# ethnhe/PVN3D

Measured on NVIDIA H100. Metric: frames/sec, higher is better.
Workload: dtype f32 (shared-MLP operands rounded to TF32, fp32 accumulate)

## Files before the change

pvn3d_b200/csrc/mlp_tc.cu:

```cuda
#include <cuda.h>

#include "common.cuh"

namespace pvn3d {
namespace {

constexpr int kMlpBM = 128;
constexpr int kMlpEpiWarps = 4;
constexpr int kMlpProWarps = 8;
constexpr int kMlpMmaWarps = 8;
constexpr int kMlpThreads = (kMlpEpiWarps + kMlpProWarps + kMlpMmaWarps) * 32;
constexpr int kMlpMaxStages = 6;
constexpr int kMlpSmemMax = 227 * 1024;

enum : int { PRO_DENSE = 0, PRO_FP_INTERP = 2, PRO_SA_FACT = 3, PRO_FP_FACT = 4 };
enum : int { EPI_STORE = 0, EPI_MAXPOOL = 1, EPI_SUMPOOL = 2, EPI_MAXPOOL_T = 3, EPI_STORE_T = 4 };

struct MlpArgs {
  alignas(64) CUtensorMap tmap;
  int use_tma;
  const float *w;
  const float *bias;
  long long rows;
  int k_pad;
// ... 816 lines not shown
  if (!enc || (reinterpret_cast<uintptr_t>(w) & 15u)) return false;
  const cuuint64_t dims[2] = {static_cast<cuuint64_t>(k_pad), static_cast<cuuint64_t>(n_pad)};
  const cuuint64_t strides[1] = {static_cast<cuuint64_t>(k_pad) * sizeof(float)};
  const cuuint32_t box[2] = {32u, static_cast<cuuint32_t>(bn)};
  const cuuint32_t estr[2] = {1u, 1u};
  return enc(map, CU_TENSOR_MAP_DATA_TYPE_FLOAT32, 2, const_cast<float *>(w), dims, strides, box, estr,
             CU_TENSOR_MAP_INTERLEAVE_NONE, CU_TENSOR_MAP_SWIZZLE_128B, CU_TENSOR_MAP_L2_PROMOTION_L2_256B,
             CU_TENSOR_MAP_FLOAT_OOB_FILL_NONE) == CUDA_SUCCESS;
}

template <int PRO, int EPI>
int launch_mlp(MlpArgs &a, cudaStream_t st) {
  if (a.rows <= 0) return PVN3D_OK;
  if (a.k_pad <= 0 || a.k_pad % 32 || a.n_pad <= 0 || a.n_pad % 16 || (reinterpret_cast<uintptr_t>(a.w) & 15u))
    return PVN3D_ERR_INVALID_ARG;
  a.bn = mma_n(a.n_pad);
  a.acc_ld = std::max(32, a.bn);
  const size_t stage_bytes = kMlpBM * 128 + align_up(static_cast<size_t>(a.bn) * 128, 1024);
  const size_t fixed = mlp_smem_front(0, a.bn, a.acc_ld) + kMlpEpiWarps * 4096 + sizeof(MlpSmemCtl);
  int stages = static_cast<int>((kMlpSmemMax - fixed) / stage_bytes);
  if (stages > kMlpMaxStages) stages = kMlpMaxStages;
  if (stages < 3) return PVN3D_ERR_UNSUPPORTED;
  a.stages = stages;
  const size_t smem = mlp_smem_front(stages, a.bn, a.acc_ld) + kMlpEpiWarps * 4096 + sizeof(MlpSmemCtl);
  a.use_tma = weight_tensor_map(&a.tmap, a.w, a.k_pad, a.n_pad, a.bn) ? 1 : 0;
  const int sms = std::max(1, sm_count() - a.reserve_sms);
  const long long tiles = ((a.rows + kMlpBM - 1) / kMlpBM) * ceil_div(a.n_pad, a.bn);
  auto kern = mlp_layer_kernel<PRO, EPI>;
  static PerDeviceOnce once;
  PVN3D_ONCE_PER_DEVICE(once, cudaFuncSetAttribute(kern, cudaFuncAttributeMaxDynamicSharedMemorySize, kMlpSmemMax),
                        "mlp smem attr");
  const unsigned grid = static_cast<unsigned>(std::min<long long>(tiles, sms));
  kern<<<grid, kMlpThreads, smem, st>>>(a);
  return check_launch("mlp_layer_kernel");
}

constexpr int kSa2Threads = (kMlpProWarps + kMlpMmaWarps) * 32;
constexpr int kSa2MaxStages = 8;
constexpr uint32_t kSa2StageBytes = kMlpBM * 128u;

struct Sa2Args {
  MlpArgs a;
  const float *w3, *bias3;
  int k3_pad, n3_pad;
};

struct Sa2SmemCtl {
  uint64_t full[kSa2MaxStages];
  uint64_t empty[kSa2MaxStages];
};

struct Sa2Smem {
  uint32_t w2, w3, h, ring, xchg, ctl, bytes;
};
static inline __host__ __device__ Sa2Smem sa2_smem(int k2_pad, int n2, int k3_pad, int n3, int stages) {
  Sa2Smem s;
  s.w2 = 0;
  s.w3 = s.w2 + static_cast<uint32_t>(k2_pad / 32) * static_cast<uint32_t>(n2) * 128u;
  s.h = s.w3 + static_cast<uint32_t>(k3_pad / 32) * static_cast<uint32_t>(n3) * 128u;
  s.ring = s.h + static_cast<uint32_t>(k3_pad / 32) * kMlpBM * 128u;
  s.xchg = s.ring + static_cast<uint32_t>(stages) * kSa2StageBytes;
  s.ctl = s.xchg + 4u * static_cast<uint32_t>(n3 > 32 ? n3 : 32) * 4u;
  s.bytes = 1024u + s.ctl + static_cast<uint32_t>(sizeof(Sa2SmemCtl));
  return s;
}

__device__ __forceinline__ void named_bar_sync(int id, int threads) {
  asm volatile("bar.sync %0, %1;" ::"r"(id), "r"(threads) : "memory");
}
__device__ __forceinline__ void named_bar_arrive(int id, int threads) {
  asm volatile("bar.arrive %0, %1;" ::"r"(id), "r"(threads) : "memory");
}

__device__ __forceinline__ void stage_weights(uint32_t dst, const float *w, int rows, int k_pad, int n) {
  const int per_chunk = n * 8;
  for (int i = threadIdx.x; i < (k_pad / 32) * per_chunk; i += blockDim.x) {
    const int kc = i / per_chunk, r = (i - kc * per_chunk) >> 3, c = i & 7;
    const float4 v = r < rows ? ldg128(w + static_cast<size_t>(r) * k_pad + kc * 32 + c * 4) : make_float4(0.f, 0.f, 0.f, 0.f);
    sts128(dst + static_cast<uint32_t>(kc * per_chunk) * 16u + sw128_off(r, c), v.x, v.y, v.z, v.w);
  }
}

template <int N2>
__device__ __forceinline__ void sa2_layer2(const Sa2Args &g, uint32_t ring, uint32_t w2_s, uint32_t h_s, int S,
                                           int it_base, int kc2, Sa2SmemCtl &ctl, unsigned wg, int frag_row,
                                           unsigned lane) {
  float d[N2 / 2];
#pragma unroll
  for (int i = 0; i < N2 / 2; ++i) d[i] = 0.f;
  int prev = -1;
  for (int kc = 0; kc < kc2; ++kc) {
    const int it = it_base + kc;
    const int s = it % S;
    mbar_wait(&ctl.full[s], static_cast<unsigned>((it / S) & 1));
    fence_proxy_async_smem();
    const uint64_t adesc = smem_desc_sw128(ring + static_cast<uint32_t>(s) * kSa2StageBytes + wg * 8192u);
    const uint64_t bdesc = smem_desc_sw128(w2_s + static_cast<uint32_t>(kc * N2) * 128u);
    wgmma_fence();
#pragma unroll
    for (int k4 = 0; k4 < 4; ++k4)
      wgmma_tf32<N2>(d, adesc + static_cast<uint64_t>(k4 * 2), bdesc + static_cast<uint64_t>(k4 * 2), (kc > 0 || k4 > 0) ? 1u : 0u);
    wgmma_commit();
    if (prev >= 0) {
      wgmma_wait<1>();
      if (lane == 0) mbar_arrive(&ctl.empty[prev]);
    }
    prev = s;
  }
  wgmma_wait<0>();
  acc_fence(d);
  if (lane == 0) mbar_arrive(&ctl.empty[prev]);
  named_bar_sync(1 + static_cast<int>(wg), 128);
  const int n2 = g.a.n_pad;
#pragma unroll
  for (int j = 0; j < N2 / 8; ++j) {
    if (8 * j >= g.k3_pad) break;
    const int c = 8 * j + 2 * static_cast<int>(lane & 3u);
    const float b0 = c < n2 ? __ldg(g.a.bias + c) : 0.f, b1 = c + 1 < n2 ? __ldg(g.a.bias + c + 1) : 0.f;
    const uint32_t off = static_cast<uint32_t>(c >> 5) * (kMlpBM * 128u) + static_cast<uint32_t>(frag_row) * 128u +
                         ((static_cast<uint32_t>(((c & 31) >> 2) ^ (frag_row & 7))) << 4) + (c & 3) * 4u;
    asm volatile("st.shared.v2.f32 [%0], {%1,%2};" ::"r"(h_s + off), "f"(to_tf32(fmaxf(d[4 * j] + b0, 0.f))),
                 "f"(to_tf32(fmaxf(d[4 * j + 1] + b1, 0.f)))
                 : "memory");
    asm volatile("st.shared.v2.f32 [%0], {%1,%2};" ::"r"(h_s + off + 8u * 128u), "f"(to_tf32(fmaxf(d[4 * j + 2] + b0, 0.f))),
                 "f"(to_tf32(fmaxf(d[4 * j + 3] + b1, 0.f)))
                 : "memory");
  }
  fence_proxy_async_smem();
  named_bar_sync(1 + static_cast<int>(wg), 128);
}

template <int HALF, int O, int NV>
__device__ __forceinline__ void rowmax_level(float (&p)[NV], unsigned lane) {
  if constexpr (HALF >= 1) {
    const bool hi = (lane & static_cast<unsigned>(O)) != 0;
#pragma unroll
    for (int i = 0; i < HALF; ++i) {
      const float keep = hi ? p[i + HALF] : p[i];
      const float send = hi ? p[i] : p[i + HALF];
      p[i] = fmaxf(keep, __shfl_xor_sync(0xffffffffu, send, O));
    }
  } else {
    p[0] = fmaxf(p[0], __shfl_xor_sync(0xffffffffu, p[0], O));
  }
}

template <int N3>
__global__ void __launch_bounds__(kSa2Threads, 1) mlp_sa_fact2_kernel(const __grid_constant__ Sa2Args g) {
  const MlpArgs &a = g.a;
  extern __shared__ unsigned char mlp_smem_raw[];
  const uint32_t raw = smem_u32(mlp_smem_raw);
  const uint32_t base = (raw + 1023u) & ~1023u;
  const int n2_mma = mma_n(a.n_pad);
  const int kc2 = a.k_pad / 32, kc3 = g.k3_pad / 32;
  const int S = a.stages;
  const Sa2Smem L = sa2_smem(a.k_pad, n2_mma, g.k3_pad, N3, S);
  Sa2SmemCtl &ctl = *reinterpret_cast<Sa2SmemCtl *>(mlp_smem_raw + (base - raw) + L.ctl);
  const int t = threadIdx.x;
  const unsigned warp = t >> 5, lane = t & 31u;
  const int tiles = static_cast<int>((a.rows + kMlpBM - 1) / kMlpBM);

  stage_weights(base + L.w2, a.w, a.n_pad, a.k_pad, n2_mma);
  stage_weights(base + L.w3, g.w3, g.n3_pad, g.k3_pad, N3);
  for (uint32_t i = t; i < static_cast<uint32_t>(kc3) * kMlpBM * 8u; i += kSa2Threads) sts128(base + L.h + i * 16u, 0.f, 0.f, 0.f, 0.f);
  if (t == 0) {
    for (int s = 0; s < S; ++s) {
      mbar_init(&ctl.full[s], 128);
      mbar_init(&ctl.empty[s], kMlpMmaWarps);
    }
    mbar_fence_init();
  }
  fence_proxy_async_smem();
  __syncthreads();

  if (warp < kMlpProWarps) {
    const int pt = t & 127;
    const unsigned grp = warp >> 2;
    const int pw = pt >> 5, sub = static_cast<int>(lane & 7u), rg = static_cast<int>(lane >> 3);
    const int r_first = 32 * pw + rg;
    int it_base = 0;
    for (int tile = blockIdx.x; tile < tiles; tile += gridDim.x, it_base += kc2) {
      if (kc2 == 1 && static_cast<unsigned>(it_base & 1) != grp) continue;
      const long long p_first = static_cast<long long>(tile) * kMlpBM + r_first;
      RowState rs;
      rows_setup<PRO_SA_FACT>(a, p_first, rs);
      for (int kc = 0; kc < kc2; ++kc) {
        const int it = it_base + kc;
        if (static_cast<unsigned>(it & 1) != grp) continue;
        const int s = static_cast<int>(it % S);
        mbar_wait(&ctl.empty[s], static_cast<unsigned>(((it / S) & 1) ^ 1));
        stage_a_chunk<PRO_SA_FACT>(a, rs, p_first, r_first, sub, kc * 32, base + L.ring + static_cast<uint32_t>(s) * kSa2StageBytes,
                                   true);
        fence_proxy_async_smem();
        mbar_arrive(&ctl.full[s]);
      }
    }
  } else {
    const unsigned mw = warp - kMlpProWarps, wg = mw >> 2, w4 = mw & 3u;
    const int frag_row = static_cast<int>(64 * wg + 16 * w4 + (lane >> 2));
    const uint32_t h_wg = base + L.h + wg * 8192u;
    const uint32_t xchg = base + L.xchg + (wg * 2u + (w4 >> 1)) * ((N3 > 32 ? N3 : 32) * 4u);
    constexpr int NV = N3 / 4;
    constexpr int NF = NV >= 8 ? NV / 8 : 1;
    int it_base = 0;
    for (int tile = blockIdx.x; tile < tiles; tile += gridDim.x, it_base += kc2) {
      const long long p0 = static_cast<long long>(tile) * kMlpBM;
      if (n2_mma == 16) sa2_layer2<16>(g, base + L.ring, base + L.w2, base + L.h, S, it_base, kc2, ctl, wg, frag_row, lane);
      else if (n2_mma == 32) sa2_layer2<32>(g, base + L.ring, base + L.w2, base + L.h, S, it_base, kc2, ctl, wg, frag_row, lane);
      else if (n2_mma == 64) sa2_layer2<64>(g, base + L.ring, base + L.w2, base + L.h, S, it_base, kc2, ctl, wg, frag_row, lane);
      else sa2_layer2<128>(g, base + L.ring, base + L.w2, base + L.h, S, it_base, kc2, ctl, wg, frag_row, lane);
      float d[N3 / 2];
#pragma unroll
      for (int i = 0; i < N3 / 2; ++i) d[i] = 0.f;
      wgmma_fence();
      for (int kc = 0; kc < kc3; ++kc) {
        const uint64_t adesc = smem_desc_sw128(h_wg + static_cast<uint32_t>(kc) * (kMlpBM * 128u));
        const uint64_t bdesc = smem_desc_sw128(base + L.w3 + static_cast<uint32_t>(kc * N3) * 128u);
#pragma unroll
        for (int k4 = 0; k4 < 4; ++k4)
          wgmma_tf32<N3>(d, adesc + static_cast<uint64_t>(k4 * 2), bdesc + static_cast<uint64_t>(k4 * 2), (kc > 0 || k4 > 0) ? 1u : 0u);
      }
      wgmma_commit();
      wgmma_wait<0>();
      acc_fence(d);
      float p[NV];
#pragma unroll
      for (int j = 0; j < N3 / 8; ++j) {
        p[2 * j] = fmaxf(d[4 * j], d[4 * j + 2]);
        p[2 * j + 1] = fmaxf(d[4 * j + 1], d[4 * j + 3]);
      }
      rowmax_level<NV / 2, 16>(p, lane);
      rowmax_level<NV / 4, 8>(p, lane);
      rowmax_level<NV / 8, 4>(p, lane);
      bool owner = true;
      long long grow = (p0 + 64 * wg + 16 * w4) / 16;
      if (a.pool == 32) {
        if (w4 & 1u) {
#pragma unroll
          for (int i = 0; i < NF; ++i)
            asm volatile("st.shared.f32 [%0], %1;" ::"r"(xchg + (lane * NF + i) * 4u), "f"(p[i]) : "memory");
          named_bar_arrive(3 + static_cast<int>(wg * 2 + (w4 >> 1)), 64);
          owner = false;
        } else {
          named_bar_sync(3 + static_cast<int>(wg * 2 + (w4 >> 1)), 64);
#pragma unroll
          for (int i = 0; i < NF; ++i) {
            float q;
            asm volatile("ld.shared.f32 %0, [%1];" : "=f"(q) : "r"(xchg + (lane * NF + i) * 4u) : "memory");
            p[i] = fmaxf(p[i], q);
          }
        }
        grow = (p0 + 64 * wg + 32 * (w4 >> 1)) / 32;
      }
      if (owner && grow * a.pool < a.rows && (NV >= 8 || !(lane & 4u))) {
        const unsigned b4 = (lane >> 4) & 1u, b3 = (lane >> 3) & 1u, b2 = (lane >> 2) & 1u;
        float *o = a.out + grow * a.ldo + a.col0;
#pragma unroll
        for (int i = 0; i < NF; ++i) {
          const int io = i + (b4 ? NV / 2 : 0) + (b3 && NV >= 4 ? NV / 4 : 0) + (b2 && NV >= 8 ? NV / 8 : 0);
          const int col = 8 * (io >> 1) + 2 * static_cast<int>(lane & 3u) + (io & 1);
          if (col < g.n3_pad) {
            float r = fmaxf(p[i] + __ldg(g.bias3 + col), 0.f);
            if (a.round_out) r = to_tf32(r);
            o[col] = r;
          }
        }
      }
    }
  }
}

int sa2_stages(int k2_pad, int n2_pad, int k3_pad, int n3_pad, int ns) {
  if ((ns != 16 && ns != 32) || n2_pad > 128 || n3_pad > 128) return 0;
  const uint32_t fixed = sa2_smem(k2_pad, mma_n(n2_pad), k3_pad, mma_n(n3_pad), 0).bytes;
  if (fixed >= static_cast<uint32_t>(kMlpSmemMax)) return 0;
  const int stages = std::min<int>(kSa2MaxStages, static_cast<int>((kMlpSmemMax - fixed) / kSa2StageBytes));
  return stages >= 2 ? stages : 0;
}

template <int N3>
int launch_sa_fact2(Sa2Args &g, int stages, cudaStream_t st) {
  MlpArgs &a = g.a;
  if (a.rows <= 0) return PVN3D_OK;
  a.stages = stages;
  const size_t smem = sa2_smem(a.k_pad, mma_n(a.n_pad), g.k3_pad, N3, stages).bytes;
  const int sms = std::max(1, sm_count() - a.reserve_sms);
  const long long tiles = (a.rows + kMlpBM - 1) / kMlpBM;
  if (tiles * (a.k_pad / 32) > 0x7fffffffll) return PVN3D_ERR_UNSUPPORTED;
  auto kern = mlp_sa_fact2_kernel<N3>;
  static PerDeviceOnce once;
  PVN3D_ONCE_PER_DEVICE(once, cudaFuncSetAttribute(kern, cudaFuncAttributeMaxDynamicSharedMemorySize, kMlpSmemMax),
                        "mlp sa_fact2 smem attr");
  const unsigned grid = static_cast<unsigned>(std::min<long long>(tiles, sms));
  kern<<<grid, kSa2Threads, smem, st>>>(g);
  return check_launch("mlp_sa_fact2_kernel");
}

constexpr int kSa2wBM = 64;
constexpr int kSa2wProWarps = 4;
constexpr int kSa2wLoaderWarp = kSa2wProWarps + kMlpMmaWarps;
constexpr int kSa2wThreads = (kSa2wLoaderWarp + 1) * 32;
constexpr int kSa2wMaxStages = 8;
constexpr int kSa2wMaxKc2 = 8;
constexpr uint32_t kSa2wChunk = kSa2wBM * 128u;
constexpr uint32_t kSa2wStageBytes = 128u * 128u;

struct Sa2wArgs {
  MlpArgs a;
  alignas(64) CUtensorMap tmap3;
  const float *w3, *bias3;
  int k3_pad, n3_pad;
};

struct Sa2wSmemCtl {
  uint64_t full[kSa2wMaxStages];
  uint64_t empty[kSa2wMaxStages];
  uint64_t a_full[kSa2wMaxKc2];
  uint64_t a_empty;
};

struct Sa2wSmem {
  uint32_t a, h, ring, ctl, bytes;
};
static inline __host__ __device__ Sa2wSmem sa2w_smem(int k2_pad, int k3_pad, int stages) {
  Sa2wSmem s;
  s.a = 0;
  s.h = s.a + static_cast<uint32_t>(k2_pad / 32) * kSa2wChunk;
  s.ring = s.h + static_cast<uint32_t>(k3_pad / 32) * kSa2wChunk;
  s.ctl = s.ring + static_cast<uint32_t>(stages) * kSa2wStageBytes;
  s.bytes = 1024u + s.ctl + static_cast<uint32_t>(sizeof(Sa2wSmemCtl));
  return s;
}

__device__ __forceinline__ int sa2w_pair_blocks(int nb, int pp) { return nb - pp < 2 ? nb - pp : 2; }

__device__ __forceinline__ int sa2w_block(float (&d)[64], uint32_t a_tile, uint32_t ring, int S, int it0, int step, int kcs,
                                          uint64_t *full, uint64_t *empty, uint64_t *a_bars, unsigned a_par, bool keep_last,
                                          unsigned lane) {
#pragma unroll
  for (int i = 0; i < 64; ++i) d[i] = 0.f;
  int prev = -1;
  for (int kc = 0; kc < kcs; ++kc) {
    const int it = it0 + kc * step;
    const int s = it % S;
    if (a_bars) mbar_wait(&a_bars[kc], a_par);
    mbar_wait(&full[s], static_cast<unsigned>((it / S) & 1));
    fence_proxy_async_smem();
    const uint64_t adesc = smem_desc_sw128(a_tile + static_cast<uint32_t>(kc) * kSa2wChunk);
    const uint64_t bdesc = smem_desc_sw128(ring + static_cast<uint32_t>(s) * kSa2wStageBytes);
    wgmma_fence();
#pragma unroll
    for (int k4 = 0; k4 < 4; ++k4)
      wgmma_tf32<128>(d, adesc + static_cast<uint64_t>(k4 * 2), bdesc + static_cast<uint64_t>(k4 * 2), (kc > 0 || k4 > 0) ? 1u : 0u);
    wgmma_commit();
    if (prev >= 0) {
      wgmma_wait<1>();
      if (lane == 0) mbar_arrive(&empty[prev]);
    }
    prev = s;
  }
  wgmma_wait<0>();
  acc_fence(d);
  if (lane == 0 && !keep_last) mbar_arrive(&empty[prev]);
  return prev;
}

__global__ void __launch_bounds__(kSa2wThreads, 1) mlp_sa_fact2w_kernel(const __grid_constant__ Sa2wArgs g) {
  const MlpArgs &a = g.a;
  extern __shared__ unsigned char mlp_smem_raw[];
  const uint32_t raw = smem_u32(mlp_smem_raw);
  const uint32_t base = (raw + 1023u) & ~1023u;
  const int kc2 = a.k_pad / 32, kc3 = g.k3_pad / 32;
  const int nb2 = (a.n_pad + 127) / 128, nb3 = (g.n3_pad + 127) / 128;
  const int S = a.stages;
  const Sa2wSmem L = sa2w_smem(a.k_pad, g.k3_pad, S);
  Sa2wSmemCtl &ctl = *reinterpret_cast<Sa2wSmemCtl *>(mlp_smem_raw + (base - raw) + L.ctl);
  const int t = threadIdx.x;
  const unsigned warp = t >> 5, lane = t & 31u;
  const int tiles = static_cast<int>((a.rows + kSa2wBM - 1) / kSa2wBM);

  if (t == 0) {
    for (int s = 0; s < S; ++s) {
      mbar_init(&ctl.full[s], 1);
      mbar_init(&ctl.empty[s], 4);
    }
    for (int kc = 0; kc < kc2; ++kc) mbar_init(&ctl.a_full[kc], 64);
    mbar_init(&ctl.a_empty, kMlpMmaWarps);
    mbar_fence_init();
  }
  __syncthreads();

  if (warp < kSa2wProWarps) {
    const int rb = static_cast<int>(warp & 1u), kc_first = static_cast<int>(warp >> 1);
    const int sub = static_cast<int>(lane & 7u), r_first = 32 * rb + static_cast<int>(lane >> 3);
    int j = 0;
    for (int tile = blockIdx.x; tile < tiles; tile += gridDim.x, ++j) {
      const long long p_first = static_cast<long long>(tile) * kSa2wBM + r_first;
      RowState rs;
      rows_setup<PRO_SA_FACT>(a, p_first, rs);
      mbar_wait(&ctl.a_empty, static_cast<unsigned>((j & 1) ^ 1));
      for (int kc = kc_first; kc < kc2; kc += 2) {
        stage_a_chunk<PRO_SA_FACT>(a, rs, p_first, r_first, sub, kc * 32, base + L.a + static_cast<uint32_t>(kc) * kSa2wChunk,
                                   true);
        fence_proxy_async_smem();
        mbar_arrive(&ctl.a_full[kc]);
      }
    }
  } else if (warp == kSa2wLoaderWarp) {
    if (lane == 0) {
      int it = 0;
      for (int tile = blockIdx.x; tile < tiles; tile += gridDim.x) {
        for (int layer = 0; layer < 2; ++layer) {
          const CUtensorMap *map = layer ? &g.tmap3 : &a.tmap;
          const int nb = layer ? nb3 : nb2, kcs = layer ? kc3 : kc2;
          for (int pp = 0; pp < nb; pp += 2) {
            const int cnt = sa2w_pair_blocks(nb, pp);
            for (int kc = 0; kc < kcs; ++kc)
              for (int q = 0; q < cnt; ++q, ++it) {
                const int s = it % S;
                mbar_wait(&ctl.empty[s], static_cast<unsigned>(((it / S) & 1) ^ 1));
                mbar_expect_tx(&ctl.full[s], kSa2wStageBytes);
                tma_load_2d(base + L.ring + static_cast<uint32_t>(s) * kSa2wStageBytes, map, kc * 32, (pp + q) * 128,
                            &ctl.full[s]);
              }
          }
        }
      }
    }
  } else {
    const unsigned mw = warp - kSa2wProWarps, wg = mw >> 2, w4 = mw & 3u;
    const int frag_row = static_cast<int>(16 * w4 + (lane >> 2));
    const int pair_bar = 2 + static_cast<int>(wg * 2 + (w4 >> 1));
    const int n2 = a.n_pad;
    int it_base = 0;
    float d[64];
    int j = 0;
    for (int tile = blockIdx.x; tile < tiles; tile += gridDim.x, ++j) {
      const long long p0 = static_cast<long long>(tile) * kSa2wBM;
      bool synced = false;
      for (int pp = 0; pp < nb2; pp += 2) {
        const int cnt = sa2w_pair_blocks(nb2, pp);
        if (static_cast<int>(wg) < cnt) {
          const int nb = pp + static_cast<int>(wg);
          float b2v[32];
#pragma unroll
          for (int jj = 0; jj < 16; ++jj) {
            const int c = 128 * nb + 8 * jj + 2 * static_cast<int>(lane & 3u);
            b2v[2 * jj] = c < n2 ? __ldg(a.bias + c) : 0.f;
            b2v[2 * jj + 1] = c + 1 < n2 ? __ldg(a.bias + c + 1) : 0.f;
          }
          sa2w_block(d, base + L.a, base + L.ring, S, it_base + static_cast<int>(wg), cnt, kc2, ctl.full, ctl.empty, ctl.a_full,
                     static_cast<unsigned>(j & 1), false, lane);
          if (!synced) named_bar_sync(1, 2 * 128);
          synced = true;
#pragma unroll
          for (int jj = 0; jj < 16; ++jj) {
            const int c = 128 * nb + 8 * jj + 2 * static_cast<int>(lane & 3u);
            if (c >= g.k3_pad) break;
            const bool on0 = c < n2, on1 = c + 1 < n2;
            const float b0 = b2v[2 * jj], b1 = b2v[2 * jj + 1];
            const uint32_t off = static_cast<uint32_t>(c >> 5) * kSa2wChunk + static_cast<uint32_t>(frag_row) * 128u +
                                 ((static_cast<uint32_t>(((c & 31) >> 2) ^ (frag_row & 7))) << 4) + (c & 3) * 4u;
            asm volatile("st.shared.v2.f32 [%0], {%1,%2};" ::"r"(base + L.h + off),
                         "f"(on0 ? to_tf32(fmaxf(d[4 * jj] + b0, 0.f)) : 0.f), "f"(on1 ? to_tf32(fmaxf(d[4 * jj + 1] + b1, 0.f)) : 0.f)
                         : "memory");
            asm volatile("st.shared.v2.f32 [%0], {%1,%2};" ::"r"(base + L.h + off + 8u * 128u),
                         "f"(on0 ? to_tf32(fmaxf(d[4 * jj + 2] + b0, 0.f)) : 0.f),
                         "f"(on1 ? to_tf32(fmaxf(d[4 * jj + 3] + b1, 0.f)) : 0.f)
                         : "memory");
          }
        }
        it_base += kc2 * cnt;
      }
      if (lane == 0) mbar_arrive(&ctl.a_empty);
      if (!synced) named_bar_sync(1, 2 * 128);
      fence_proxy_async_smem();
      named_bar_sync(1, 2 * 128);
      for (int pp = 0; pp < nb3; pp += 2) {
        const int cnt = sa2w_pair_blocks(nb3, pp);
        if (static_cast<int>(wg) < cnt) {
          const int nb = pp + static_cast<int>(wg);
          const unsigned b4 = (lane >> 4) & 1u, b3 = (lane >> 3) & 1u, b2 = (lane >> 2) & 1u;
          float b3v[4];
#pragma unroll
          for (int i = 0; i < 4; ++i) {
            const int io = i + (b4 ? 16 : 0) + (b3 ? 8 : 0) + (b2 ? 4 : 0);
            const int col = 128 * nb + 8 * (io >> 1) + 2 * static_cast<int>(lane & 3u) + (io & 1);
            b3v[i] = col < g.n3_pad ? __ldg(g.bias3 + col) : 0.f;
          }
          const int last = sa2w_block(d, base + L.h, base + L.ring, S, it_base + static_cast<int>(wg), cnt, kc3, ctl.full, ctl.empty, nullptr, 0u,
                                      true, lane);
          float p[32];
#pragma unroll
          for (int jj = 0; jj < 16; ++jj) {
            p[2 * jj] = fmaxf(d[4 * jj], d[4 * jj + 2]);
            p[2 * jj + 1] = fmaxf(d[4 * jj + 1], d[4 * jj + 3]);
          }
          rowmax_level<16, 16>(p, lane);
          rowmax_level<8, 8>(p, lane);
          rowmax_level<4, 4>(p, lane);
          bool owner = true;
          long long grow = (p0 + 16 * w4) / 16;
          if (a.pool == 32) {
            const uint32_t xc = base + L.ring + static_cast<uint32_t>(last) * kSa2wStageBytes + (w4 >> 1) * 512u;
            if (w4 & 1u) {
#pragma unroll
              for (int i = 0; i < 4; ++i)
                asm volatile("st.shared.f32 [%0], %1;" ::"r"(xc + (lane * 4 + i) * 4u), "f"(p[i]) : "memory");
              fence_proxy_async_smem();
              named_bar_sync(pair_bar, 64);
              owner = false;
            } else {
              named_bar_sync(pair_bar, 64);
#pragma unroll
              for (int i = 0; i < 4; ++i) {
                float q;
                asm volatile("ld.shared.f32 %0, [%1];" : "=f"(q) : "r"(xc + (lane * 4 + i) * 4u) : "memory");
                p[i] = fmaxf(p[i], q);
              }
            }
            grow = (p0 + 32 * (w4 >> 1)) / 32;
          }
          __syncwarp();
          if (lane == 0) mbar_arrive(&ctl.empty[last]);
          if (owner && grow * a.pool < a.rows) {
            float *o = a.out + grow * a.ldo + a.col0;
#pragma unroll
            for (int i = 0; i < 4; ++i) {
              const int io = i + (b4 ? 16 : 0) + (b3 ? 8 : 0) + (b2 ? 4 : 0);
              const int col = 128 * nb + 8 * (io >> 1) + 2 * static_cast<int>(lane & 3u) + (io & 1);
              if (col < g.n3_pad) {
                float r = fmaxf(p[i] + b3v[i], 0.f);
                if (a.round_out) r = to_tf32(r);
                o[col] = r;
              }
            }
          }
        }
        it_base += kc3 * cnt;
      }
    }
  }
}

int sa2w_stages(int k2_pad, int n2_pad, int k3_pad, int n3_pad, int ns) {
  if ((ns != 16 && ns != 32) || n3_pad <= 128 || k2_pad / 32 > kSa2wMaxKc2 || k3_pad > 128 * ceil_div(n2_pad, 128)) return 0;
  const uint32_t fixed = sa2w_smem(k2_pad, k3_pad, 0).bytes;
  if (fixed >= static_cast<uint32_t>(kMlpSmemMax)) return 0;
  const int stages = std::min<int>(kSa2wMaxStages, static_cast<int>((kMlpSmemMax - fixed) / kSa2wStageBytes));
  return stages >= 3 ? stages : 0;
}

int launch_sa_fact2w(Sa2wArgs &g, int stages, cudaStream_t st) {
  MlpArgs &a = g.a;
  if (a.rows <= 0) return PVN3D_OK;
  a.stages = stages;
  const size_t smem = sa2w_smem(a.k_pad, g.k3_pad, stages).bytes;
  const int sms = std::max(1, sm_count() - a.reserve_sms);
  const long long tiles = (a.rows + kSa2wBM - 1) / kSa2wBM;
  const long long chunks = static_cast<long long>(ceil_div(a.n_pad, 128)) * (a.k_pad / 32) +
                           static_cast<long long>(ceil_div(g.n3_pad, 128)) * (g.k3_pad / 32);
  if (tiles * chunks > 0x7fffffffll) return PVN3D_ERR_UNSUPPORTED;
  if (!weight_tensor_map(&a.tmap, a.w, a.k_pad, a.n_pad, 128) || !weight_tensor_map(&g.tmap3, g.w3, g.k3_pad, g.n3_pad, 128))
    return PVN3D_ERR_UNSUPPORTED;
  auto kern = mlp_sa_fact2w_kernel;
  static PerDeviceOnce once;
  PVN3D_ONCE_PER_DEVICE(once, cudaFuncSetAttribute(kern, cudaFuncAttributeMaxDynamicSharedMemorySize, kMlpSmemMax),
                        "mlp sa_fact2w smem attr");
  const unsigned grid = static_cast<unsigned>(std::min<long long>(tiles, sms));
  kern<<<grid, kSa2wThreads, smem, st>>>(g);
  return check_launch("mlp_sa_fact2w_kernel");
}

constexpr int kFp2BM = 64;
constexpr int kFp2ProWarps = 4;
constexpr int kFp2Pairs = kFp2ProWarps / 2;
constexpr int kFp2LoaderWarp = kFp2ProWarps + kMlpMmaWarps;
constexpr int kFp2Threads = (kFp2LoaderWarp + 1) * 32;
constexpr int kFp2MaxStages = 8;
constexpr uint32_t kFp2AStageBytes = kFp2BM * 128u;
constexpr uint32_t kFp2WStageBytes = 128u * 128u;

struct Fp2Args {
  MlpArgs a;
  alignas(64) CUtensorMap tmap2;
  const float *w2, *bias2;
  int k2_pad, n2_pad;
  int a_stages, w_stages;
};

struct Fp2SmemCtl {
  uint64_t a_full[kFp2MaxStages];
  uint64_t a_empty[kFp2MaxStages];
  uint64_t w_full[kFp2MaxStages];
  uint64_t w_empty[kFp2MaxStages];
};

struct Fp2Smem {
  uint32_t h, aring, wring, rows, ctl, bytes;
};
static inline __host__ __device__ Fp2Smem fp2_smem(int k2_pad, int a_stages, int w_stages) {
  Fp2Smem s;
  s.h = 0;
  s.aring = s.h + static_cast<uint32_t>(k2_pad / 32) * kFp2AStageBytes;
  s.wring = s.aring + static_cast<uint32_t>(a_stages) * kFp2AStageBytes;
  s.rows = s.wring + static_cast<uint32_t>(w_stages) * kFp2WStageBytes;
  s.ctl = s.rows + kFp2ProWarps * 32u * 32u;
  s.bytes = 1024u + s.ctl + static_cast<uint32_t>(sizeof(Fp2SmemCtl));
  return s;
}

__device__ __forceinline__ void fp2_rows_store(const RowState &rs, uint32_t rst, unsigned sub) {
  if (sub != 0) return;
#pragma unroll
  for (int j = 0; j < 8; ++j) {
    asm volatile("st.shared.v4.s32 [%0], {%1,%2,%3,%4};" ::"r"(rst + 128u * j), "r"(rs.g1[j]), "r"(rs.g2[j]), "r"(rs.g3[j]), "r"(0)
                 : "memory");
    sts128(rst + 128u * j + 16u, rs.w1[j], rs.w2[j], rs.w3[j], ((rs.live >> j) & 1u) ? 1.f : 0.f);
  }
}
__device__ __forceinline__ int4 lds128i(uint32_t addr) {
  int4 v;
  asm volatile("ld.shared.v4.s32 {%0,%1,%2,%3}, [%4];" : "=r"(v.x), "=r"(v.y), "=r"(v.z), "=r"(v.w) : "r"(addr));
  return v;
}

__device__ __forceinline__ void fp2_stage_chunk(const MlpArgs &a, uint32_t rst, long long p_first, int r_first, int sub,
                                                int k0, uint32_t sa, bool vec_ok) {
  const int k = k0 + 4 * sub;
  const float4 zero = make_float4(0.f, 0.f, 0.f, 0.f);
  if (vec_ok && k + 4 <= a.c2) {
    const float *kf = a.known_feat + k;
#pragma unroll
    for (int h = 0; h < 2; ++h) {
      float4 p1[4], p2[4], p3[4];
#pragma unroll
      for (int jj = 0; jj < 4; ++jj) {
        const int4 gi = lds128i(rst + 128u * (h * 4 + jj));
        p1[jj] = ldg128(kf + static_cast<size_t>(gi.x) * a.c2);
        p2[jj] = ldg128(kf + static_cast<size_t>(gi.y) * a.c2);
        p3[jj] = ldg128(kf + static_cast<size_t>(gi.z) * a.c2);
      }
#pragma unroll
      for (int jj = 0; jj < 4; ++jj) {
        const int j = h * 4 + jj;
        const float4 w = lds128(rst + 128u * j + 16u);
        float4 v;
        v.x = __fmaf_rn(p3[jj].x, w.z, __fmaf_rn(p1[jj].x, w.x, __fmul_rn(p2[jj].x, w.y)));
        v.y = __fmaf_rn(p3[jj].y, w.z, __fmaf_rn(p1[jj].y, w.x, __fmul_rn(p2[jj].y, w.y)));
        v.z = __fmaf_rn(p3[jj].z, w.z, __fmaf_rn(p1[jj].z, w.x, __fmul_rn(p2[jj].z, w.y)));
        v.w = __fmaf_rn(p3[jj].w, w.z, __fmaf_rn(p1[jj].w, w.x, __fmul_rn(p2[jj].w, w.y)));
        if (w.w == 0.f) v = zero;
        sts_tf32(sa + sw128_off(r_first + 4 * j, sub), v);
      }
    }
    return;
  }
  const bool skip_vec = (a.c2 % 4 == 0) && (a.lds % 4 == 0) && ((reinterpret_cast<uintptr_t>(a.skip) & 15u) == 0);
  if (skip_vec && k >= a.c2 && k - a.c2 + 4 <= a.c1) {
    float4 v[8];
#pragma unroll
    for (int j = 0; j < 8; ++j)
      v[j] = lds128(rst + 128u * j + 16u).w != 0.f ? ldg128(a.skip + (p_first + 4 * j) * a.lds + (k - a.c2)) : zero;
#pragma unroll
    for (int j = 0; j < 8; ++j) sts_tf32(sa + sw128_off(r_first + 4 * j, sub), v[j]);
    return;
  }
  if (k >= a.c2 + a.c1) {
#pragma unroll
    for (int j = 0; j < 8; ++j) sts128(sa + sw128_off(r_first + 4 * j, sub), 0.f, 0.f, 0.f, 0.f);
    return;
  }
#pragma unroll
  for (int j = 0; j < 8; ++j) {
    const int4 gi = lds128i(rst + 128u * j);
    const float4 w = lds128(rst + 128u * j + 16u);
    const bool live = w.w != 0.f;
    const long long p = p_first + 4 * j;
    float vv[4];
#pragma unroll
    for (int e = 0; e < 4; ++e) {
      const int kk = k + e;
      const bool isk = live && kk < a.c2;
      const int d = kk - a.c2;
      const bool iss = live && d >= 0 && d < a.c1;
      const float *kf = a.known_feat + (isk ? kk : 0);
      const float p1 = isk ? __ldg(kf + static_cast<size_t>(gi.x) * a.c2) : 0.f;
      const float p2 = isk ? __ldg(kf + static_cast<size_t>(gi.y) * a.c2) : 0.f;
      const float p3 = isk ? __ldg(kf + static_cast<size_t>(gi.z) * a.c2) : 0.f;
      const float sk = iss ? __ldg(a.skip + p * a.lds + (iss ? d : 0)) : 0.f;
      vv[e] = isk ? __fmaf_rn(p3, w.z, __fmaf_rn(p1, w.x, __fmul_rn(p2, w.y))) : sk;
    }
    sts_tf32(sa + sw128_off(r_first + 4 * j, sub), make_float4(vv[0], vv[1], vv[2], vv[3]));
  }
}

__device__ __forceinline__ void fp2_layer1_block(float (&d)[64], uint32_t aring, uint32_t wring, int SA, int SW, int ita0,
                                                 int itw0, int kc1, Fp2SmemCtl &ctl, unsigned lane) {
#pragma unroll
  for (int i = 0; i < 64; ++i) d[i] = 0.f;
  int pa = -1, pw = -1;
  for (int kc = 0; kc < kc1; ++kc) {
    const int ita = ita0 + kc, itw = itw0 + 2 * kc;
    const int sa = ita % SA, sw = itw % SW;
    mbar_wait(&ctl.a_full[sa], static_cast<unsigned>((ita / SA) & 1));
    mbar_wait(&ctl.w_full[sw], static_cast<unsigned>((itw / SW) & 1));
    fence_proxy_async_smem();
    const uint64_t adesc = smem_desc_sw128(aring + static_cast<uint32_t>(sa) * kFp2AStageBytes);
    const uint64_t bdesc = smem_desc_sw128(wring + static_cast<uint32_t>(sw) * kFp2WStageBytes);
    wgmma_fence();
#pragma unroll
    for (int k4 = 0; k4 < 4; ++k4)
      wgmma_tf32<128>(d, adesc + static_cast<uint64_t>(k4 * 2), bdesc + static_cast<uint64_t>(k4 * 2), (kc > 0 || k4 > 0) ? 1u : 0u);
    wgmma_commit();
    if (pa >= 0) {
      wgmma_wait<1>();
      if (lane == 0) {
        mbar_arrive(&ctl.a_empty[pa]);
        mbar_arrive(&ctl.w_empty[pw]);
      }
    }
    pa = sa;
    pw = sw;
  }
  wgmma_wait<0>();
  acc_fence(d);
  if (lane == 0) {
    mbar_arrive(&ctl.a_empty[pa]);
    mbar_arrive(&ctl.w_empty[pw]);
  }
}

__global__ void __launch_bounds__(kFp2Threads, 1) mlp_fp2_kernel(const __grid_constant__ Fp2Args g) {
  const MlpArgs &a = g.a;
  extern __shared__ unsigned char mlp_smem_raw[];
  const uint32_t raw = smem_u32(mlp_smem_raw);
  const uint32_t base = (raw + 1023u) & ~1023u;
  const int kc1 = a.k_pad / 32, kc2 = g.k2_pad / 32;
  const int nb1 = a.n_pad / 128, nb2 = g.n2_pad / 128;
  const int SA = g.a_stages, SW = g.w_stages;
  const Fp2Smem L = fp2_smem(g.k2_pad, SA, SW);
  Fp2SmemCtl &ctl = *reinterpret_cast<Fp2SmemCtl *>(mlp_smem_raw + (base - raw) + L.ctl);
  const int t = threadIdx.x;
  const unsigned warp = t >> 5, lane = t & 31u;
  const int tiles = static_cast<int>((a.rows + kFp2BM - 1) / kFp2BM);

  if (t == 0) {
    for (int s = 0; s < SA; ++s) {
      mbar_init(&ctl.a_full[s], 64);
      mbar_init(&ctl.a_empty[s], kMlpMmaWarps);
    }
    for (int s = 0; s < SW; ++s) {
      mbar_init(&ctl.w_full[s], 1);
      mbar_init(&ctl.w_empty[s], 4);
    }
    mbar_fence_init();
  }
  __syncthreads();

  if (warp < kFp2ProWarps) {
    const unsigned pair = warp >> 1;
    const int sub = static_cast<int>(lane & 7u), r_first = 32 * static_cast<int>(warp & 1u) + static_cast<int>(lane >> 3);
    const bool vec_ok = (a.c2 % 4 == 0) && ((reinterpret_cast<uintptr_t>(a.known_feat) & 15u) == 0);
    const int per_tile = (nb1 / 2) * kc1;
    const uint32_t rst = base + L.rows + warp * 1024u + (lane >> 3) * 32u;
    int it = 0;
    for (int tile = blockIdx.x; tile < tiles; tile += gridDim.x) {
      const long long p_first = static_cast<long long>(tile) * kFp2BM + r_first;
      {
        RowState rs;
        rows_setup<PRO_FP_INTERP>(a, p_first, rs);
        __syncwarp();
        fp2_rows_store(rs, rst, static_cast<unsigned>(sub));
        __syncwarp();
      }
      for (int i = 0; i < per_tile; ++i, ++it) {
        if (static_cast<unsigned>(it % kFp2Pairs) != pair) continue;
        const int s = it % SA;
        mbar_wait(&ctl.a_empty[s], static_cast<unsigned>(((it / SA) & 1) ^ 1));
        const int kc = i % kc1;
        fp2_stage_chunk(a, rst, p_first, r_first, sub, kc * 32, base + L.aring + static_cast<uint32_t>(s) * kFp2AStageBytes, vec_ok);
        fence_proxy_async_smem();
        mbar_arrive(&ctl.a_full[s]);
      }
    }
  } else if (warp == kFp2LoaderWarp) {
    if (lane == 0) {
      int it = 0;
      for (int tile = blockIdx.x; tile < tiles; tile += gridDim.x) {
        for (int layer = 0; layer < 2; ++layer) {
          const CUtensorMap *map = layer ? &g.tmap2 : &a.tmap;
          const int nb = layer ? nb2 : nb1, kcs = layer ? kc2 : kc1;
          for (int pp = 0; pp < nb; pp += 2) {
            const int cnt = sa2w_pair_blocks(nb, pp);
            for (int kc = 0; kc < kcs; ++kc)
              for (int q = 0; q < cnt; ++q, ++it) {
                const int s = it % SW;
                mbar_wait(&ctl.w_empty[s], static_cast<unsigned>(((it / SW) & 1) ^ 1));
                mbar_expect_tx(&ctl.w_full[s], kFp2WStageBytes);
                tma_load_2d(base + L.wring + static_cast<uint32_t>(s) * kFp2WStageBytes, map, kc * 32, (pp + q) * 128,
                            &ctl.w_full[s]);
              }
          }
        }
      }
    }
  } else {
    const unsigned mw = warp - kFp2ProWarps, wg = mw >> 2, w4 = mw & 3u;
    const int frag_row = static_cast<int>(16 * w4 + (lane >> 2));
    const uint32_t h_s = base + L.h;
    int ita = 0, itw = 0;
    float d[64];
    for (int tile = blockIdx.x; tile < tiles; tile += gridDim.x) {
      const long long p0 = static_cast<long long>(tile) * kFp2BM;
      for (int pp = 0; pp < nb1; pp += 2) {
        const int nb = pp + static_cast<int>(wg);
        fp2_layer1_block(d, base + L.aring, base + L.wring, SA, SW, ita, itw + static_cast<int>(wg), kc1, ctl, lane);
        ita += kc1;
        itw += 2 * kc1;
        if (pp == 0) named_bar_sync(1, 2 * 128);
#pragma unroll
        for (int jj = 0; jj < 16; ++jj) {
          const int c = 128 * nb + 8 * jj + 2 * static_cast<int>(lane & 3u);
          const float b0 = __ldg(a.bias + c), b1 = __ldg(a.bias + c + 1);
          const uint32_t off = static_cast<uint32_t>(c >> 5) * kFp2AStageBytes + static_cast<uint32_t>(frag_row) * 128u +
                               ((static_cast<uint32_t>(((c & 31) >> 2) ^ (frag_row & 7))) << 4) + (c & 3) * 4u;
          asm volatile("st.shared.v2.f32 [%0], {%1,%2};" ::"r"(h_s + off), "f"(to_tf32(fmaxf(d[4 * jj] + b0, 0.f))),
                       "f"(to_tf32(fmaxf(d[4 * jj + 1] + b1, 0.f)))
                       : "memory");
          asm volatile("st.shared.v2.f32 [%0], {%1,%2};" ::"r"(h_s + off + 8u * 128u), "f"(to_tf32(fmaxf(d[4 * jj + 2] + b0, 0.f))),
                       "f"(to_tf32(fmaxf(d[4 * jj + 3] + b1, 0.f)))
                       : "memory");
        }
      }
      fence_proxy_async_smem();
      named_bar_sync(1, 2 * 128);
      const long long r0 = p0 + frag_row;
      for (int pp = 0; pp < nb2; pp += 2) {
        const int cnt = sa2w_pair_blocks(nb2, pp);
        if (static_cast<int>(wg) < cnt) {
          const int nb = pp + static_cast<int>(wg);
          sa2w_block(d, h_s, base + L.wring, SW, itw + static_cast<int>(wg), cnt, kc2, ctl.w_full, ctl.w_empty, nullptr, 0u,
                     false, lane);
          float *o = a.out + r0 * a.ldo + a.col0 + 128 * nb + 2 * static_cast<int>(lane & 3u);
          const bool on0 = r0 < a.rows, on1 = r0 + 8 < a.rows;
#pragma unroll
          for (int jj = 0; jj < 16; ++jj) {
            const int c = 128 * nb + 8 * jj + 2 * static_cast<int>(lane & 3u);
            const float b0 = __ldg(g.bias2 + c), b1 = __ldg(g.bias2 + c + 1);
// ... 628 lines not shown
```

Before: 6129.

## Replace fused two-layer MLP barriers with per-chunk mbarrier handoff between warpgroups

Restructures the fused SA two-layer MLP kernel so the two MMA warpgroups alternate over individual output blocks (units) of both layers, ordered by a turn mbarrier. Named-barrier syncs and the single A-tile empty barrier are replaced by per-k-chunk A release, per-block hidden-ready barriers and an h_empty barrier. Layer-3 work can then start as soon as the needed hidden chunks are written, and the producer can refill A chunks early. The cost is more mbarrier traffic and serialized turn handoffs. A new cap on layer-2 output blocks also limits which shapes take this path.

Result: faster. 6202, median of 6 (+1.2%).

```diff
diff --git a/pvn3d_b200/csrc/mlp_tc.cu b/pvn3d_b200/csrc/mlp_tc.cu
--- a/pvn3d_b200/csrc/mlp_tc.cu
+++ b/pvn3d_b200/csrc/mlp_tc.cu
@@ -1142,6 +1142,7 @@
 constexpr int kSa2wThreads = (kSa2wLoaderWarp + 1) * 32;
 constexpr int kSa2wMaxStages = 8;
 constexpr int kSa2wMaxKc2 = 8;
+constexpr int kSa2wMaxNb2 = 8;
 constexpr uint32_t kSa2wChunk = kSa2wBM * 128u;
 constexpr uint32_t kSa2wStageBytes = 128u * 128u;
 
@@ -1156,7 +1157,10 @@
   uint64_t full[kSa2wMaxStages];
   uint64_t empty[kSa2wMaxStages];
   uint64_t a_full[kSa2wMaxKc2];
-  uint64_t a_empty;
+  uint64_t a_empty[kSa2wMaxKc2];
+  uint64_t h_full[kSa2wMaxNb2];
+  uint64_t h_empty;
+  uint64_t turn[2];
 };
 
 struct Sa2wSmem {
@@ -1202,6 +1206,43 @@
   wgmma_wait<0>();
   acc_fence(d);
   if (lane == 0 && !keep_last) mbar_arrive(&empty[prev]);
+  return prev;
+}
+
+__device__ __forceinline__ int sa2w_unit(float (&d)[64], uint32_t a_tile, uint32_t ring, int S, int it0, int kcs,
+                                         uint64_t *full, uint64_t *empty, uint64_t *ready, int rshift, unsigned rpar,
+                                         uint64_t *a_rel, uint64_t *my_turn, int turn_par, uint64_t *next_turn,
+                                         unsigned lane) {
+#pragma unroll
+  for (int i = 0; i < 64; ++i) d[i] = 0.f;
+  if (turn_par >= 0) mbar_wait(my_turn, static_cast<unsigned>(turn_par));
+  int prev = -1;
+  for (int kc = 0; kc < kcs; ++kc) {
+    const int it = it0 + kc;
+    const int s = it % S;
+    mbar_wait(&ready[kc >> rshift], rpar);
+    mbar_wait(&full[s], static_cast<unsigned>((it / S) & 1));
+    if (kc == kcs - 1 && lane == 0) mbar_arrive(next_turn);
+    fence_proxy_async_smem();
+    const uint64_t adesc = smem_desc_sw128(a_tile + static_cast<uint32_t>(kc) * kSa2wChunk);
+    const uint64_t bdesc = smem_desc_sw128(ring + static_cast<uint32_t>(s) * kSa2wStageBytes);
+    wgmma_fence();
+#pragma unroll
+    for (int k4 = 0; k4 < 4; ++k4)
+      wgmma_tf32<128>(d, adesc + static_cast<uint64_t>(k4 * 2), bdesc + static_cast<uint64_t>(k4 * 2), (kc > 0 || k4 > 0) ? 1u : 0u);
+    wgmma_commit();
+    if (prev >= 0) {
+      wgmma_wait<1>();
+      if (lane == 0) {
+        mbar_arrive(&empty[prev]);
+        if (a_rel) mbar_arrive(&a_rel[kc - 1]);
+      }
+    }
+    prev = s;
+  }
+  wgmma_wait<0>();
+  acc_fence(d);
+  if (lane == 0 && a_rel) mbar_arrive(&a_rel[kcs - 1]);
   return prev;
 }
 
@@ -1224,8 +1265,14 @@
       mbar_init(&ctl.full[s], 1);
       mbar_init(&ctl.empty[s], 4);
     }
-    for (int kc = 0; kc < kc2; ++kc) mbar_init(&ctl.a_full[kc], 64);
-    mbar_init(&ctl.a_empty, kMlpMmaWarps);
+    for (int kc = 0; kc < kc2; ++kc) {
+      mbar_init(&ctl.a_full[kc], 64);
+      mbar_init(&ctl.a_empty[kc], 4 * nb2);
+    }
+    for (int nb = 0; nb < nb2; ++nb) mbar_init(&ctl.h_full[nb], 128);
+    mbar_init(&ctl.h_empty, 4 * nb3);
+    mbar_init(&ctl.turn[0], 4);
+    mbar_init(&ctl.turn[1], 4);
     mbar_fence_init();
   }
   __syncthreads();
@@ -1238,8 +1285,8 @@
       const long long p_first = static_cast<long long>(tile) * kSa2wBM + r_first;
       RowState rs;
       rows_setup<PRO_SA_FACT>(a, p_first, rs);
-      mbar_wait(&ctl.a_empty, static_cast<unsigned>((j & 1) ^ 1));
       for (int kc = kc_first; kc < kc2; kc += 2) {
+        mbar_wait(&ctl.a_empty[kc], static_cast<unsigned>((j & 1) ^ 1));
         stage_a_chunk<PRO_SA_FACT>(a, rs, p_first, r_first, sub, kc * 32, base + L.a + static_cast<uint32_t>(kc) * kSa2wChunk,
                                    true);
         fence_proxy_async_smem();
@@ -1250,19 +1297,15 @@
     if (lane == 0) {
       int it = 0;
       for (int tile = blockIdx.x; tile < tiles; tile += gridDim.x) {
-        for (int layer = 0; layer < 2; ++layer) {
-          const CUtensorMap *map = layer ? &g.tmap3 : &a.tmap;
-          const int nb = layer ? nb3 : nb2, kcs = layer ? kc3 : kc2;
-          for (int pp = 0; pp < nb; pp += 2) {
-            const int cnt = sa2w_pair_blocks(nb, pp);
-            for (int kc = 0; kc < kcs; ++kc)
-              for (int q = 0; q < cnt; ++q, ++it) {
-                const int s = it % S;
-                mbar_wait(&ctl.empty[s], static_cast<unsigned>(((it / S) & 1) ^ 1));
-                mbar_expect_tx(&ctl.full[s], kSa2wStageBytes);
-                tma_load_2d(base + L.ring + static_cast<uint32_t>(s) * kSa2wStageBytes, map, kc * 32, (pp + q) * 128,
-                            &ctl.full[s]);
-              }
+        for (int un = 0; un < nb2 + nb3; ++un) {
+          const bool l3 = un >= nb2;
+          const CUtensorMap *map = l3 ? &g.tmap3 : &a.tmap;
+          const int nb = l3 ? un - nb2 : un, kcs = l3 ? kc3 : kc2;
+          for (int kc = 0; kc < kcs; ++kc, ++it) {
+            const int s = it % S;
+            mbar_wait(&ctl.empty[s], static_cast<unsigned>(((it / S) & 1) ^ 1));
+            mbar_expect_tx(&ctl.full[s], kSa2wStageBytes);
+            tma_load_2d(base + L.ring + static_cast<uint32_t>(s) * kSa2wStageBytes, map, kc * 32, nb * 128, &ctl.full[s]);
           }
         }
       }
@@ -1272,16 +1315,17 @@
     const int frag_row = static_cast<int>(16 * w4 + (lane >> 2));
     const int pair_bar = 2 + static_cast<int>(wg * 2 + (w4 >> 1));
     const int n2 = a.n_pad;
-    int it_base = 0;
     float d[64];
-    int j = 0;
-    for (int tile = blockIdx.x; tile < tiles; tile += gridDim.x, ++j) {
-      const long long p0 = static_cast<long long>(tile) * kSa2wBM;
-      bool synced = false;
-      for (int pp = 0; pp < nb2; pp += 2) {
-        const int cnt = sa2w_pair_blocks(nb2, pp);
-        if (static_cast<int>(wg) < cnt) {
-          const int nb = pp + static_cast<int>(wg);
+    for (int j = 0; static_cast<int>(blockIdx.x + j * gridDim.x) < tiles; ++j) {
+      const unsigned par = static_cast<unsigned>(j & 1);
+      for (int un = 0; un < nb2 + nb3; ++un) {
+        const int u = j * (nb2 + nb3) + un;
+        if ((u & 1) != static_cast<int>(wg)) continue;
+        const bool l3 = un >= nb2;
+        const int it0 = j * (nb2 * kc2 + nb3 * kc3) + (l3 ? nb2 * kc2 + (un - nb2) * kc3 : un * kc2);
+        const int turn_par = u > 0 ? ((u - 1) >> 1) & 1 : -1;
+        if (!l3) {
+          const int nb = un;
           float b2v[32];
 #pragma unroll
           for (int jj = 0; jj < 16; ++jj) {
@@ -1289,10 +1333,10 @@
             b2v[2 * jj] = c < n2 ? __ldg(a.bias + c) : 0.f;
             b2v[2 * jj + 1] = c + 1 < n2 ? __ldg(a.bias + c + 1) : 0.f;
           }
-          sa2w_block(d, base + L.a, base + L.ring, S, it_base + static_cast<int>(wg), cnt, kc2, ctl.full, ctl.empty, ctl.a_full,
-                     static_cast<unsigned>(j & 1), false, lane);
-          if (!synced) named_bar_sync(1, 2 * 128);
-          synced = true;
+          const int last = sa2w_unit(d, base + L.a, base + L.ring, S, it0, kc2, ctl.full, ctl.empty, ctl.a_full, 0, par,
+                                     ctl.a_empty, &ctl.turn[u & 1], turn_par, &ctl.turn[(u + 1) & 1], lane);
+          if (lane == 0) mbar_arrive(&ctl.empty[last]);
+          mbar_wait(&ctl.h_empty, par ^ 1u);
 #pragma unroll
           for (int jj = 0; jj < 16; ++jj) {
             const int c = 128 * nb + 8 * jj + 2 * static_cast<int>(lane & 3u);
@@ -1309,17 +1353,10 @@
                          "f"(on1 ? to_tf32(fmaxf(d[4 * jj + 3] + b1, 0.f)) : 0.f)
                          : "memory");
           }
-        }
-        it_base += kc2 * cnt;
-      }
-      if (lane == 0) mbar_arrive(&ctl.a_empty);
-      if (!synced) named_bar_sync(1, 2 * 128);
-      fence_proxy_async_smem();
-      named_bar_sync(1, 2 * 128);
-      for (int pp = 0; pp < nb3; pp += 2) {
-        const int cnt = sa2w_pair_blocks(nb3, pp);
-        if (static_cast<int>(wg) < cnt) {
-          const int nb = pp + static_cast<int>(wg);
+          fence_proxy_async_smem();
+          mbar_arrive(&ctl.h_full[nb]);
+        } else {
+          const int nb = un - nb2;
           const unsigned b4 = (lane >> 4) & 1u, b3 = (lane >> 3) & 1u, b2 = (lane >> 2) & 1u;
           float b3v[4];
 #pragma unroll
@@ -1328,8 +1365,9 @@
             const int col = 128 * nb + 8 * (io >> 1) + 2 * static_cast<int>(lane & 3u) + (io & 1);
             b3v[i] = col < g.n3_pad ? __ldg(g.bias3 + col) : 0.f;
           }
-          const int last = sa2w_block(d, base + L.h, base + L.ring, S, it_base + static_cast<int>(wg), cnt, kc3, ctl.full, ctl.empty, nullptr, 0u,
-                                      true, lane);
+          const int last = sa2w_unit(d, base + L.h, base + L.ring, S, it0, kc3, ctl.full, ctl.empty, ctl.h_full, 2, par,
+                                     nullptr, &ctl.turn[u & 1], turn_par, &ctl.turn[(u + 1) & 1], lane);
+          if (lane == 0) mbar_arrive(&ctl.h_empty);
           float p[32];
 #pragma unroll
           for (int jj = 0; jj < 16; ++jj) {
@@ -1340,6 +1378,7 @@
           rowmax_level<8, 8>(p, lane);
           rowmax_level<4, 4>(p, lane);
           bool owner = true;
+          const long long p0 = static_cast<long long>(blockIdx.x + j * gridDim.x) * kSa2wBM;
           long long grow = (p0 + 16 * w4) / 16;
           if (a.pool == 32) {
             const uint32_t xc = base + L.ring + static_cast<uint32_t>(last) * kSa2wStageBytes + (w4 >> 1) * 512u;
@@ -1377,14 +1416,15 @@
             }
           }
         }
-        it_base += kc3 * cnt;
       }
     }
   }
 }
 
 int sa2w_stages(int k2_pad, int n2_pad, int k3_pad, int n3_pad, int ns) {
-  if ((ns != 16 && ns != 32) || n3_pad <= 128 || k2_pad / 32 > kSa2wMaxKc2 || k3_pad > 128 * ceil_div(n2_pad, 128)) return 0;
+  if ((ns != 16 && ns != 32) || n3_pad <= 128 || k2_pad / 32 > kSa2wMaxKc2 || ceil_div(n2_pad, 128) > kSa2wMaxNb2 ||
+      k3_pad > 128 * ceil_div(n2_pad, 128))
+    return 0;
   const uint32_t fixed = sa2w_smem(k2_pad, k3_pad, 0).bytes;
   if (fixed >= static_cast<uint32_t>(kMlpSmemMax)) return 0;
   const int stages = std::min<int>(kSa2wMaxStages, static_cast<int>((kMlpSmemMax - fixed) / kSa2wStageBytes));
```
